# olydis/vlg_matching

Hardware: AMD Instinct MI355X
Metric: vlg_queries_per_sec (higher is better)
Workload: dtype u32

## Files before the change

### vlg_matching_amd/csrc/join_device.hpp

```cpp
#pragma once
#include "doc_cut.hpp"
namespace {

constexpr uint32_t kNone = 0xFFFFFFFFu;
constexpr uint32_t kChecksumSlots = 64;

struct SegMeta {
    uint32_t begin, end;
    uint32_t pbegin, pend;
    uint32_t dist;
    uint32_t level;
    uint32_t next;
    uint32_t query;
    uint64_t lo, hi;
};

struct QueryMeta {
    uint32_t seg0;
    uint32_t k;
    uint64_t end_len;
    uint64_t out_first;
    uint64_t out_tuple;
};

// ... 42 lines not shown
{
    RungLayout L{};
    L.levels = 0;
    while (L.levels < kMaxRungs && (total >> (kRungShift * (L.levels + 1))) != 0) ++L.levels;
    uint64_t at = 0;
    for (uint32_t j = 1; j <= L.levels; ++j) {
        L.off[j] = at;
        at += (((total >> (kRungShift * j)) + kRungFan - 1) & ~(uint64_t)(kRungFan - 1)) + kRungFan;
    }
    L.entries = at;
    return L;
}

template <typename pos_t>
__global__ void rung_build_kernel(const pos_t* __restrict__ P, uint64_t total, pos_t* __restrict__ R, const uint64_t* __restrict__ off, uint32_t levels,
                                  pos_t* __restrict__ F)
{
    for (uint64_t i = (uint64_t)blockIdx.x * blockDim.x + threadIdx.x; i < (total >> kRungShift); i += (uint64_t)gridDim.x * blockDim.x) {
        const pos_t v = P[kRungFan * i + kRungFan - 1];
        R[off[1] + i] = v;
        uint64_t k = i;
        for (uint32_t j = 2; j <= levels && (k & (kRungFan - 1)) == kRungFan - 1; ++j) {
            k >>= kRungShift;
            R[off[j] + k] = v;
            if (F && kRungShift * j == 6) F[k] = v;
        }
    }
}
constexpr bool kRungsHoldFences = 6 % kRungShift == 0 && kRungShift < 6;

template <typename pos_t> struct alignas(4 * sizeof(pos_t)) RungQuad { pos_t v[4]; };

constexpr uint32_t kFarRounds = 4;
template <typename pos_t>
__device__ __forceinline__ void wave_far_lower_bound(const pos_t* __restrict__ P, const pos_t* __restrict__ F, uint32_t wb, uint32_t b, pos_t key,
                                                     bool need, uint32_t& j, pos_t& val)
{
    const uint32_t lane = threadIdx.x & 63;
    constexpr pos_t kInf = (pos_t)~(pos_t)0;
    for (uint32_t round = 0; round < kFarRounds && wb < b; ++round) {
        if (!__any(need)) return;
        const uint32_t g0 = F ? wb >> 6 : 0;
        pos_t f;
        if (F) f = g0 + lane < (b >> 6) ? F[g0 + lane] : kInf;
        else { const uint64_t fi = (uint64_t)wb + 64 * lane + 63; f = fi < b ? P[fi] : kInf; }
        const pos_t flast = __shfl(f, 63);
        const bool can = need && key <= flast;
        uint32_t lo = 0;
#pragma unroll
        for (uint32_t step = 32; step; step >>= 1) {
            const pos_t v = __shfl(f, (int)(lo + step - 1));
            lo += v < key ? step : 0u;
        }
        if (can) {
            uint64_t w0 = F ? ((uint64_t)(g0 + lo) << 6) : (uint64_t)wb + 64 * lo;
            const uint64_t w1 = w0 + 64 < b ? w0 + 64 : b;
            if (w0 < wb) w0 = wb;
            uint32_t pos = 0;
#pragma unroll
            for (uint32_t step = 32; step; step >>= 1) {
                const uint64_t at = w0 + pos + step - 1;
                if (at < w1 && P[at] < key) pos += step;
            }
            const uint64_t at = w0 + pos;
            if (at < b) { j = (uint32_t)at; val = P[at]; } else j = b;
            need = false;
        }
        const uint64_t nwb = F ? ((uint64_t)(g0 + 64) << 6) : (uint64_t)wb + 4096;
        wb = nwb < b ? (uint32_t)nwb : b;
    }
    if (need) {
        j = gallop_lower_bound(P, wb < b ? wb : b, b, (uint64_t)key);
        if (j < b) val = P[j]; else j = b;
    }
// ... 1 lines not shown

constexpr uint32_t kCoopWindows = 4;
template <typename pos_t>
__device__ __forceinline__ uint32_t wave_lower_bound(const pos_t* __restrict__ P, const pos_t* __restrict__ F, uint32_t wb, uint32_t b, pos_t key, bool need, pos_t& val)
{
    const uint32_t lane = threadIdx.x & 63;
    constexpr pos_t kInf = (pos_t)~(pos_t)0;
    uint32_t res = b;
    for (uint32_t it = 0; it < kCoopWindows; ++it) {
        if (!__any(need)) break;
        const uint32_t idx = wb + lane;
        const pos_t w = idx < b ? P[idx] : kInf;
        const pos_t wlast = __shfl(w, 63);
        const bool can = need && key <= wlast;
        uint32_t lo = 0;
#pragma unroll
        for (uint32_t step = 32; step; step >>= 1) {
            const pos_t v = __shfl(w, (int)(lo + step - 1));
            lo += v < key ? step : 0u;
        }
        const pos_t at = __shfl(w, (int)lo);
        if (can) { res = wb + lo; val = at; need = false; }
        wb += 64;
    }
    if (__any(need)) wave_far_lower_bound(P, F, wb < b ? wb : b, b, key, need, res, val);
    return res < b ? res : b;
}

#ifndef VLG_COOP_WINDOWS2
#define VLG_COOP_WINDOWS2 4
#endif
static_assert(VLG_COOP_WINDOWS2 >= 1, "VLG_COOP_WINDOWS2: at least one window before the far search");
constexpr uint32_t kCoopWindows2 = VLG_COOP_WINDOWS2;
template <typename pos_t>
__device__ __forceinline__ void wave_lower_bound2(const pos_t* __restrict__ P, const pos_t* __restrict__ F, uint32_t wb, uint32_t b, pos_t key0, bool need0, pos_t key1,
                                                  bool need1, uint32_t& j0, pos_t& v0, uint32_t& j1, pos_t& v1)
{
    const uint32_t lane = threadIdx.x & 63;
    constexpr pos_t kInf = (pos_t)~(pos_t)0;
    j0 = b; j1 = b;
    for (uint32_t it = 0; it < kCoopWindows2; ++it) {
        if (!__any(need0 || need1)) break;
        const uint32_t idx = wb + lane;
        const pos_t w = idx < b ? P[idx] : kInf;
        const pos_t wlast = __shfl(w, 63);
        const bool can0 = need0 && key0 <= wlast, can1 = need1 && key1 <= wlast;
        uint32_t lo0 = 0, lo1 = 0;
#pragma unroll
        for (uint32_t step = 32; step; step >>= 1) {
            const pos_t a0 = __shfl(w, (int)(lo0 + step - 1)), a1 = __shfl(w, (int)(lo1 + step - 1));
            lo0 += a0 < key0 ? step : 0u;
            lo1 += a1 < key1 ? step : 0u;
        }
        const pos_t at0 = __shfl(w, (int)lo0), at1 = __shfl(w, (int)lo1);
        if (can0) { j0 = wb + lo0; v0 = at0; need0 = false; }
        if (can1) { j1 = wb + lo1; v1 = at1; need1 = false; }
        wb += 64;
    }
    if (__any(need0 || need1)) {
        wb = wb < b ? wb : b;
        wave_far_lower_bound(P, F, wb, b, key0, need0, j0, v0);
        wave_far_lower_bound(P, F, wb, b, key1, need1, j1, v1);
    }
}

constexpr uint32_t kKeys = 8;
constexpr uint32_t kBlk = 64 * kKeys;
constexpr uint32_t kTB = 1024;
constexpr uint32_t kKeyGroup = 4;
constexpr uint32_t kMinPiece = 128;

__device__ __forceinline__ void wave_sync()
{
    __builtin_amdgcn_fence(__ATOMIC_ACQ_REL, "wavefront");
    __builtin_amdgcn_wave_barrier();
}

template <typename T>
__device__ __forceinline__ T wave_min(T v)
{
    for (int o = 32; o > 0; o >>= 1) { const T u = __shfl_xor(v, o); v = u < v ? u : v; }
    return v;
}

template <typename T>
__device__ __forceinline__ T wave_max(T v)
{
    for (int o = 32; o > 0; o >>= 1) { const T u = __shfl_xor(v, o); v = u > v ? u : v; }
    return v;
}
template <typename T>
__device__ __forceinline__ T wave_or(T v)
{
    for (int o = 32; o > 0; o >>= 1) v |= __shfl_xor(v, o);
    return v;
// ... 380 lines not shown
    pos_t x_pre = 0, x_pre1 = 0;
    bool have_pre = false, have_pre1 = false;
    for (uint32_t base = run_begin; base < run_end; base += 64) {
        if (base >= seg_end) {
            while (seg_begin[s_w + 1] <= base) ++s_w;
            seg_end = seg_begin[s_w + 1];
            m = sm[s_w]; nx = sm[m.next];
            lvl0 = kJump && m.level == 0;
            end_len = lvl0 ? qm[m.query].end_len : 0;
            if (kDocs) { m_len = dr.seg_len[s_w]; m_next = dr.seg_len[m.next]; }
            have_pre = false; have_pre1 = false;
        }
        if (run_end - base >= 128 && base + 127 < seg_end) {
            const uint32_t e0 = base + lane, e1 = e0 + 64;
            const pos_t x0 = have_pre ? x_pre : P[phys_of(m, e0)];
            const pos_t x1 = have_pre1 ? x_pre1 : P[phys_of(m, e1)];
            const uint32_t left = run_end - base - 128;
            const uint32_t room = seg_end - base - 128;
            have_pre = left > 0 && (left < 64 ? left : 64u) <= room;
            have_pre1 = left >= 128 && room >= 128;
            if (lvl0) {
                x_pre = e0 + 128 < m.end ? P[phys_of(m, e0 + 128)] : kInf;
                x_pre1 = e1 + 128 < m.end ? P[phys_of(m, e1 + 128)] : kInf;
            } else {
                if (have_pre) x_pre = e0 + 128 < run_end ? P[phys_of(m, e0 + 128)] : (pos_t)0;
                if (have_pre1) x_pre1 = P[phys_of(m, e1 + 128)];
            }
            pos_t tlo0, thi0, tlo1, thi1, v0 = 0, v1 = 0;
            const bool want0 = gap_window<pos_t>((uint64_t)x0, nx.lo, nx.hi, tlo0, thi0);
            const bool want1 = gap_window<pos_t>((uint64_t)x1, nx.lo, nx.hi, tlo1, thi1);
            uint32_t j0 = nx.pend, j1 = nx.pend;
            if (hint_seg != s_w)
                hint = wave_kary_lower_bound(P, F, nx.pbegin, nx.pend, (uint64_t)__shfl(tlo0, 0));
            wave_lower_bound2(P, F, hint, nx.pend, tlo0, want0, tlo1, want1, j0, v0, j1, v1);
            if (!want0) j0 = nx.pend;
            if (!want1) j1 = nx.pend;
            bool in0 = want0, in1 = want1;
            uint64_t nb0 = 0, nb1 = 0;
            if (kDocs) {
                dw.locate(dr, (uint64_t)__shfl(x0, 0), (uint64_t)__shfl(x1, 63));
                nb0 = dw.nb(dr, (uint64_t)x0); nb1 = dw.nb(dr, (uint64_t)x1);
                in0 = want0 && doc_window<pos_t>((uint64_t)x0, m_len, m_next, nb0, thi0);
                in1 = want1 && doc_window<pos_t>((uint64_t)x1, m_len, m_next, nb1, thi1);
            }
            pos_t end0 = 0, end1 = 0;
            const bool ok0 = link_finish<pos_t, kLast>(P, nx, fb, e0, in0, j0, v0, thi0, endp, link, !lvl0, end0);
            const bool ok1 = link_finish<pos_t, kLast>(P, nx, fb, e1, in1, j1, v1, thi1, endp, link, !lvl0, end1);
            const unsigned long long okm0 = __ballot(ok0), okm1 = __ballot(ok1);
            if (lane == 0) { fbits_out[base >> 6] = okm0; fbits_out[(base >> 6) + 1] = okm1; }
            if (kJump) {
                if (lvl0) {
                    pos_t key[2] = {0, 0};
                    const bool need[2] = {ok0 && restart_key<pos_t, kDocs>((uint64_t)end0, end_len, nb0, key[0]),
                                          ok1 && restart_key<pos_t, kDocs>((uint64_t)end1, end_len, nb1, key[1])};
                    tile[lane] = x0; tile[64 + lane] = x1; tile[128 + lane] = x_pre; tile[192 + lane] = x_pre1;
                    wave_sync();
                    uint32_t out[2];
                    stretch_jump_targets<pos_t, 2>(P, F, m, phys_of(m, base), tile, key, need, out);
                    wave_sync();
                    jump[e0] = out[0]; jump[e1] = out[1];
                } else {
                    if (e0 >= jlo && e0 < jhi) jump[e0] = kNone;
                    if (e1 >= jlo && e1 < jhi) jump[e1] = kNone;
                }
            }
            hint_seg = s_w;
            hint = __shfl(j1, 63);
// ... 320 lines not shown
#pragma unroll
    for (uint32_t r = 0; r < 4; ++r) {
        const uint32_t li = threadIdx.x + 256 * r;
        const uint64_t e = base + li;
        if (e < r1) xh[e] = make_uint2(s_ext[st[r] >> 21], ((st[r] >> 11) & 1023u) + 1);
    }
}

__global__ void chain_walk_kernel(const SegMeta* __restrict__ sm, const QueryMeta* __restrict__ qm, uint32_t nq, FeasRef fb,
                                  const uint2* __restrict__ xh, const uint32_t* __restrict__ rec_begin,
                                  uint2* __restrict__ records, uint32_t* __restrict__ rec_count, unsigned long long* __restrict__ counts)
{
    uint32_t q = blockIdx.x * blockDim.x + threadIdx.x;
    if (q >= nq) return;
    const QueryMeta Q = qm[q];
    unsigned long long n_match = 0;
    uint32_t nrec = 0;
    if (Q.seg0 != kNone) {
        const uint32_t mbegin = sm[Q.seg0].begin, mend = sm[Q.seg0].end;
        uint2* rec = records + rec_begin[q];
        uint32_t cur = mbegin < mend ? next_feasible(fb, mbegin) : kNone;
        if (cur >= mend) cur = kNone;
        while (cur != kNone) {
            uint2 v = xh[cur];
            rec[nrec++] = make_uint2(cur, mbegin + (uint32_t)n_match);
            n_match += v.y;
            cur = v.x;
        }
    }
    rec_count[q] = nrec;
    counts[q] = n_match;
}

__global__ void __launch_bounds__(256) chain_emit_kernel(const uint32_t* __restrict__ rec_begin, const uint32_t* __restrict__ rec_count,
                                                         const uint2* __restrict__ records, uint32_t total_rec_slots,
                                                         const uint32_t* __restrict__ rec_query, const uint32_t* __restrict__ jump,
                                                         const uint2* __restrict__ xh, uint64_t r1 ,
                                                         uint32_t* __restrict__ mlist)
{
    constexpr uint16_t kOut = 0xFFFFu;
    constexpr uint32_t kPer = kTile / 64;
    __shared__ uint16_t s_t[4][2][kTile];
    const uint32_t lane = threadIdx.x & 63, wv = threadIdx.x >> 6;
    const uint32_t r = uniform((uint32_t)(((uint64_t)blockIdx.x * blockDim.x + threadIdx.x) >> 6));
    if (r >= total_rec_slots) return;
    const uint32_t q = rec_query[r];
    if (r - rec_begin[q] >= rec_count[q]) return;
    const uint2 rc = records[r];
    const uint64_t tile_base = (uint64_t)(rc.x / kTile) * kTile;
    const uint32_t cnt = uniform(xh[rc.x].y);
#pragma unroll
    for (uint32_t i = 0; i < kPer; ++i) {
        const uint64_t e = tile_base + lane + 64 * i;
        const uint32_t j = e < r1 ? jump[e] : kNone;
        s_t[wv][0][lane + 64 * i] = (j != kNone && (uint64_t)j < tile_base + kTile) ? (uint16_t)(j - (uint32_t)tile_base) : kOut;
    }
    wave_sync();
    uint32_t cur[kPer];
#pragma unroll
    for (uint32_t i = 0; i < kPer; ++i) cur[i] = rc.x - (uint32_t)tile_base;
    uint32_t buf = 0;
    for (uint32_t k = 0; (1u << k) < cnt; ++k) {
        const uint16_t* __restrict__ T = s_t[wv][buf];
#pragma unroll
        for (uint32_t i = 0; i < kPer; ++i) {
            const uint32_t rank = lane + 64 * i;
            if (rank < cnt && ((rank >> k) & 1)) cur[i] = T[cur[i]];
        }
        if ((2u << k) < cnt) {
            uint16_t* __restrict__ N = s_t[wv][buf ^ 1];
#pragma unroll
            for (uint32_t i = 0; i < kPer; ++i) {
                const uint32_t sl = lane + 64 * i;
                const uint16_t a = T[sl];
                N[sl] = a == kOut ? kOut : T[a];
            }
            wave_sync();
            buf ^= 1;
        }
    }
#pragma unroll
    for (uint32_t i = 0; i < kPer; ++i) {
        const uint32_t rank = lane + 64 * i;
        if (rank < cnt) mlist[rc.y + rank] = (uint32_t)tile_base + cur[i];
    }
}

template <typename pos_t>
__global__ void __launch_bounds__(256) join_gather_kernel(const pos_t* __restrict__ P, const SegMeta* __restrict__ sm, const QueryMeta* __restrict__ qm,
                                                          const unsigned long long* __restrict__ first_of , uint32_t nq,
                                                          uint64_t n_matches, const uint32_t* __restrict__ link, const uint32_t* __restrict__ mlist,
                                                          pos_t* __restrict__ out_first, pos_t* __restrict__ out_tuples, unsigned long long* __restrict__ checksum)
{
    const uint32_t lane = threadIdx.x & 63;
    const uint64_t wave = ((uint64_t)blockIdx.x * blockDim.x + threadIdx.x) >> 6;
    const uint64_t run_begin = wave * kRun;
    const bool live = run_begin < n_matches;
    const uint64_t run_end = !live ? run_begin : (run_begin + kRun < n_matches ? run_begin + kRun : n_matches);
    uint32_t q_w = 0, q_end = 0;
    if (live) {
        const uint32_t ub = wave_kary_lower_bound<unsigned long long>(first_of, 0, nq, run_begin + 1);
        q_w = uniform(ub ? ub - 1 : 0u);
        const uint32_t ue = wave_kary_lower_bound<unsigned long long>(first_of, 0, nq, run_end);
        q_end = uniform(ue ? ue - 1 : 0u);
    }
    unsigned long long local = 0;
    for (uint64_t base = run_begin; base < run_end; base += 64) {
        const uint64_t g = base + lane;
        uint32_t q = q_w;
        if (g < run_end) {
            uint32_t hi = q_end;
            while (q < hi) {
                const uint32_t mid = q + ((hi - q + 1) >> 1);
                if (first_of[mid] <= g) q = mid; else hi = mid - 1;
            }
            const QueryMeta Q = qm[q];
            const SegMeta m = sm[Q.seg0];
// ... 32 lines not shown
```

### vlg_matching_amd/csrc/search.hip

```cpp
#include <algorithm>
#include <chrono>
#include <cstdio>
#include <cstdlib>
#include <cstring>
#include <mutex>
#include <numeric>
#include <thread>
#include <unordered_map>
#include <string.h>
#include <string>
#include <vector>
#include "common.hpp"
#include "kernels.hpp"
#include <rocprim/rocprim.hpp>

using namespace vlg;

#include "search_types.hpp"
#include "filter_shape.hpp"
#include "window_cut.hpp"
#include "shape_dispatch.hpp"

enum { KS_BSEARCH = 0, KS_EXPAND, KS_LOCATE, KS_LOCATE_PART, KS_LOCATE_RESOLVE, KS_SORT, KS_FILTER_LADDER, KS_FILTER_PIVOT, KS_FILTER_PASS, KS_FILTER_COMPACT,
       KS_JOIN_INIT, KS_JOIN_LINK, KS_JOIN_SCAN, KS_JOIN_CHAIN, KS_GATHER, KS_EXCHANGE, KS_WINDOW_CUT, KS_CLASS_SEARCH, KS_COUNT };
static const char* kKernelNames[KS_COUNT] = {"backward_search", "expand", "locate", "locate_partition", "locate_resolve", "sort", "filter_ladder", "filter_pivot",
                                             "filter_pass", "filter_compact", "join_init", "join_link", "join_scan", "join_chain", "gather", "exchange", "window_cut", "class_search"};

struct vlg_workspace {
    hipStream_t stream = nullptr;
    uint64_t cap_bytes = 0;
    uint8_t* arena = nullptr;
    uint64_t arena_bytes = 0;
    HostPool host;
    bool profile = false;
    bool dedup = true;
    bool sweep = true;
    bool tuples = true;
    bool trail = true;
    bool filter = true;
    uint64_t filter_min = 1ull << 12;
    uint64_t filter_stream_min = 1ull << 16;
    bool filter_pivot = true;
    uint64_t filter_group_bytes = 0;
    uint64_t filter_pivot_ratio = 3;
    uint64_t pivot_range_ratio = 16;
    uint32_t compact_dense_min = 256;
    uint32_t pivot_rungs = 1;
    int list_sort = 1;
    uint64_t global_sort_min = 1ull << 20;
    bool quad_walk = true;
    bool fuse_jump = true;
    bool sweep_compact = true;
    uint64_t sweep_min = 1ull << 22;
    uint64_t sweep_tail = 1ull << 22;
    uint32_t unsample_pct = 0;
    uint64_t unsample_min = 1ull << 28;
    uint64_t unsample_tail = 1ull << 20;
    uint32_t class_intervals = 1024;
    uint64_t sample_reads = 0;
    uint8_t* head = nullptr;
    uint64_t head_bytes = 0;
    uint64_t tmp_key[6] = {0, 0, 0, 0, 0, 0};
    size_t tmp_bytes = 0;
    int x_ranks = 1, x_rank = 0;
    vlg_exchange_fn x_fn = nullptr;
    vlg_alltoall_fn x_a2a = nullptr;
    void* x_ctx = nullptr;
    void* x_comm = nullptr;
    bool exchange_all = false;
    uint64_t* x_status = nullptr;
    uint32_t x_agreed = 0;
    vlg_kernel_stat stats[KS_COUNT];
    std::vector<std::pair<hipEvent_t, hipEvent_t>> pending[KS_COUNT];
    std::vector<hipEvent_t> free_events;
};

namespace {

struct PhaseTrace {
    bool on, sync;
    hipStream_t st;
    std::chrono::steady_clock::time_point t0;
    explicit PhaseTrace(hipStream_t s) : on(getenv("VLG_TRACE") != nullptr), sync(!on || strcmp(getenv("VLG_TRACE"), "host") != 0), st(s), t0(std::chrono::steady_clock::now()) {}
    void mark(const char* what)
// ... 112 lines not shown

extern "C" void vlg_workspace_destroy(vlg_workspace* ws)
{
    if (!ws) return;
    ws_collect(ws);
    for (hipEvent_t e : ws->free_events) (void)hipEventDestroy(e);
    if (ws->arena) (void)hipFree(ws->arena);
    if (ws->head) (void)hipFree(ws->head);
    if (ws->x_status) (void)hipFree(ws->x_status);
    ws->host.release();
    delete ws;
}

extern "C" vlg_status vlg_workspace_profile(vlg_workspace* ws, int enable)
{
    if (!ws) return fail(VLG_E_INVALID, "null argument");
    ws_reset_stats(ws);
    ws->profile = enable != 0;
    return VLG_OK;
}

extern "C" vlg_status vlg_workspace_set_option(vlg_workspace* ws, const char* name, int64_t value)
{
    if (!ws || !name) return fail(VLG_E_INVALID, "null argument");
    if (!strcmp(name, "dedup")) { ws->dedup = value != 0; return VLG_OK; }
    if (!strcmp(name, "sweep")) { ws->sweep = value != 0; return VLG_OK; }
    if (!strcmp(name, "sweep_min")) { ws->sweep_min = (uint64_t)value; return VLG_OK; }
    if (!strcmp(name, "global_sort_min")) { ws->global_sort_min = (uint64_t)value; return VLG_OK; }
    if (!strcmp(name, "list_sort")) { ws->list_sort = value > 2 ? 1 : (int)value; return VLG_OK; }
    if (!strcmp(name, "trail")) { ws->trail = value != 0; return VLG_OK; }
    if (!strcmp(name, "quad_walk")) { ws->quad_walk = value != 0; return VLG_OK; }
    if (!strcmp(name, "tuples")) { ws->tuples = value != 0; return VLG_OK; }
    if (!strcmp(name, "fuse_jump")) { ws->fuse_jump = value != 0; return VLG_OK; }
    if (!strcmp(name, "sweep_compact")) { ws->sweep_compact = value != 0; return VLG_OK; }
    if (!strcmp(name, "filter")) { ws->filter = value != 0; return VLG_OK; }
    if (!strcmp(name, "filter_min")) { ws->filter_min = (uint64_t)value; return VLG_OK; }
    if (!strcmp(name, "filter_pivot")) { ws->filter_pivot = value != 0; return VLG_OK; }
    if (!strcmp(name, "filter_pivot_ratio")) { ws->filter_pivot_ratio = (uint64_t)value; return VLG_OK; }
    if (!strcmp(name, "pivot_range_ratio")) { ws->pivot_range_ratio = (uint64_t)std::max<int64_t>(0, value); return VLG_OK; }
    if (!strcmp(name, "compact_dense_min")) { ws->compact_dense_min = (uint32_t)std::max<int64_t>(0, std::min<int64_t>(value, 1 << 20)); return VLG_OK; }
    if (!strcmp(name, "pivot_rungs")) { ws->pivot_rungs = value <= 0 ? 0u : (value == 1 ? 1u : 2u); return VLG_OK; }
    if (!strcmp(name, "filter_stream_min")) { ws->filter_stream_min = (uint64_t)value; return VLG_OK; }
    if (!strcmp(name, "filter_group_bytes")) { ws->filter_group_bytes = (uint64_t)value; return VLG_OK; }
    if (!strcmp(name, "reserve")) {
        const uint64_t b = std::min<uint64_t>((uint64_t)value, ws->cap_bytes);
        return ws_reserve(ws, b + b / 96 + (256ull << 20));
    }
    if (!strcmp(name, "sweep_tail")) { ws->sweep_tail = (uint64_t)value; return VLG_OK; }
    if (!strcmp(name, "exchange_all")) { ws->exchange_all = value != 0; return VLG_OK; }
    if (!strcmp(name, "unsample_pct")) { ws->unsample_pct = (uint32_t)std::max<int64_t>(0, std::min<int64_t>(value, 1 << 20)); return VLG_OK; }
    if (!strcmp(name, "unsample_tail")) { ws->unsample_tail = (uint64_t)value; return VLG_OK; }
    if (!strcmp(name, "class_intervals")) {
        if (value < 1 || value > (int64_t)kClassIntervalsMax) return fail(VLG_E_INVALID, "class_intervals: 1 .. 2^20");
        ws->class_intervals = (uint32_t)value;
        return VLG_OK;
    }
    if (!strcmp(name, "unsample_min")) { ws->unsample_min = (uint64_t)value; return VLG_OK; }
    return fail(VLG_E_INVALID, std::string("unknown workspace option ") + name);
}

namespace {
vlg_status ws_exchange_reset(vlg_workspace* ws, int n_ranks)
{
    ws->x_comm = nullptr; ws->x_fn = nullptr; ws->x_a2a = nullptr; ws->x_ctx = nullptr; ws->x_ranks = 1; ws->x_rank = 0;
    if (n_ranks > 1 && !ws->x_status) VLG_HIP_TRY(hipMalloc((void**)&ws->x_status, 8 * 1024));
    return VLG_OK;
// ... 920 lines not shown
    if (vlg_status s = pp.carve()) return s;
    if (vlg_status s = pp.locate(plan_sort)) return s;
    if (vlg_status s = pp.sort(L.P)) return s;
    if (vlg_status s = pp.exchange(L.P, q, xq, ag)) return s;
    if (vlg_status s = pp.check_sort()) return s;
    if (vlg_status s = pp.fences_and_ladder()) return s;
    res->sum.located_occurrences += pp.acc;
    return VLG_OK;
}

}

#include "filter.hpp"

namespace {

inline bool fuse_jump_env() { static const bool on = [] { const char* e = getenv("VLG_FUSE_JUMP"); return !(e && e[0] == '0'); }(); return on; }

template <typename pos_t>
struct JoinChunk {
    const vlg_queries* q; vlg_workspace* ws; vlg_result* res; const uint64_t q0, q1; const Plan& pl; const Lists<pos_t>& L;
    Arena A;
    unsigned long long* d_stats; const FilterGroup* fg;
    hipStream_t st = ws->stream;
    PhaseTrace jt{st};
    const pos_t* P = L.P;
    pos_t* Pc = L.Pc;
    const pos_t* F = L.F;
    const uint64_t s0 = q->qsub[q0], s1 = q->qsub[q1];
    const uint32_t nseg = (uint32_t)(s1 - s0), nq = (uint32_t)(q1 - q0);
    ResultPiece piece{q0, q1};
    bool empty = false;
    const bool fused = ws->fuse_jump && fuse_jump_env();
    const vlg_documents* docs = q->docs;
    svec<uint64_t> seg_len; uint64_t* d_seglen = nullptr; DocRef dref{};
    svec<QueryMeta> qm;
    uint32_t kmax = 0, nlive = 0, n_rec = 0;
    svec<uint32_t> t_seg, t_cidx; svec<uint64_t> t_run0;
    bool t_kind[2] = {false, false};
    uint64_t pc_total = 0;
    std::vector<uint32_t> cls_count, cls_first;
    std::vector<uint64_t> cls_slot_begin, cls_slot_end;
    svec<SegMeta> sm; svec<uint32_t> seg_begin;
    uint64_t T = 0, lvl0_begin = 0, lvl0_end = 0, t0 = 0;
    svec<uint32_t> rec_begin, rec_query;
    svec<unsigned long long> counts, first_of;
    uint32_t* link = nullptr; pos_t* endp = nullptr;
    FeasBits fb; uint64_t* lvl_ptr[kBitLevels]; FeasBits* d_fb = nullptr; FeasRef fref{nullptr, nullptr};
    uint32_t* jump = nullptr; uint32_t* mlist = nullptr; uint2* xh = nullptr;
    SegMeta* d_sm = nullptr; QueryMeta* d_qm = nullptr; uint32_t* d_segb = nullptr; unsigned long long* d_counts = nullptr;
    uint32_t* d_recb = nullptr; uint32_t* d_recc = nullptr; uint32_t* d_recq = nullptr; uint2* d_rec = nullptr;

    uint64_t eo(uint64_t s) const { return fg ? fg->eff[s - fg->sub0] : pl.occ[s]; }
    bool filtered(uint64_t s) const { return fg && fg->cidx[s - fg->sub0] != kNone; }
    bool live(uint64_t qi) const { return q->qsub[qi + 1] > q->qsub[qi] && eo(q->qsub[qi]) > 0; }

    void survivor_tasks()
    {
        qm.resize(nq);
        if (fg) { t_seg.reserve(nseg); t_cidx.reserve(nseg); t_run0.reserve(nseg + 1); }
        t_run0.push_back(0);
        for (uint64_t qi = q0; qi < q1; ++qi) {
            const uint64_t a = q->qsub[qi];
            const uint32_t k = (uint32_t)(q->qsub[qi + 1] - a);
            QueryMeta& Q = qm[qi - q0];
            Q.k = k; Q.end_len = q->end_len[qi]; Q.out_first = Q.out_tuple = 0; Q.seg0 = kNone;
// ... 92 lines not shown
        sm[nlive] = SegMeta{(uint32_t)acc, (uint32_t)acc, 0, 0, 0, 0, kNone, 0, 0, 0};
        if (T == 0 || nlive == 0) { empty = true; return; }
        lvl0_begin = T; lvl0_end = 0;
        rec_begin.assign(nq + 1, 0);
        for (uint32_t i = 0; i < nq; ++i) {
            uint32_t cnt = 0;
            const SegMeta& m0 = sm[qm[i].seg0 != kNone ? qm[i].seg0 : nlive];
            if (m0.end > m0.begin) {
                lvl0_begin = std::min<uint64_t>(lvl0_begin, m0.begin); lvl0_end = std::max<uint64_t>(lvl0_end, m0.end);
                cnt = (m0.end - 1) / kTile - m0.begin / kTile + 1;
            }
            rec_begin[i + 1] = rec_begin[i] + cnt;
            rec_query.insert(rec_query.end(), cnt, i);
        }
        n_rec = rec_begin[nq];
        empty = lvl0_end <= lvl0_begin;
        t0 = lvl0_begin / kTile * kTile;
    }

    vlg_status carve()
    {
        link = ws->tuples ? A.take<uint32_t>(T) : nullptr;
        endp = A.take<pos_t>(T);
        uint64_t words = (T + 63) / 64 + 1;
        for (uint32_t l = 0; l < kBitLevels; ++l) {
            fb.lvl[l] = lvl_ptr[l] = A.take<uint64_t>(words);
            fb.words[l] = words;
            words = (words + 63) / 64 + 1;
        }
        d_fb = A.take<FeasBits>(1);
        fref = FeasRef{lvl_ptr[0], d_fb};
        const uint64_t n0 = lvl0_end - t0;
        uint32_t* jump_a = A.take<uint32_t>(n0);
        uint32_t* mlist_a = A.take<uint32_t>(n0);
        uint2* xh_a = A.take<uint2>(n0);
        jump = jump_a ? jump_a - t0 : nullptr;
        mlist = mlist_a ? mlist_a - t0 : nullptr;
        xh = xh_a ? xh_a - t0 : nullptr;
        d_sm = A.take<SegMeta>(nlive + 1);
        d_qm = A.take<QueryMeta>(nq);
        d_segb = A.take<uint32_t>(nlive + 2);
        if (docs) d_seglen = A.take<uint64_t>(nlive + 1);
        d_counts = A.take<unsigned long long>(nq);
        d_recb = A.take<uint32_t>(nq + 1);
        d_recc = A.take<uint32_t>(nq);
        d_recq = A.take<uint32_t>(n_rec + 1);
        d_rec = A.take<uint2>(n_rec + 1);
        if (A.failed) return fail(VLG_E_INTERNAL, "arena carve failed (join)");
        return VLG_OK;
    }

    vlg_status upload()
    {
        for (uint32_t l = 0; l < kBitLevels; ++l) VLG_HIP_TRY(hipMemsetAsync(lvl_ptr[l], 0, fb.words[l] * 8, st));
        VLG_HIP_TRY(hipMemcpyAsync(d_fb, &fb, sizeof fb, hipMemcpyHostToDevice, st));
        VLG_HIP_TRY(hipMemcpyAsync(d_recb, rec_begin.data(), (nq + 1) * 4, hipMemcpyHostToDevice, st));
        if (n_rec) VLG_HIP_TRY(hipMemcpyAsync(d_recq, rec_query.data(), n_rec * 4, hipMemcpyHostToDevice, st));
        VLG_HIP_TRY(hipMemcpyAsync(d_sm, sm.data(), (nlive + 1) * sizeof(SegMeta), hipMemcpyHostToDevice, st));
        VLG_HIP_TRY(hipMemcpyAsync(d_segb, seg_begin.data(), (nlive + 2) * 4, hipMemcpyHostToDevice, st));
        VLG_HIP_TRY(hipMemcpyAsync(d_qm, qm.data(), nq * sizeof(QueryMeta), hipMemcpyHostToDevice, st));
        if (docs) {
            VLG_HIP_TRY(hipMemcpyAsync(d_seglen, seg_len.data(), (nlive + 1) * 8, hipMemcpyHostToDevice, st));
            dref = doc_ref(docs, d_seglen);
        }
        return VLG_OK;
    }

// ... 9 lines not shown
        }
        VLG_HIP_TRY(hipGetLastError());
        return VLG_OK;
    }

    vlg_status link_classes()
    {
        if (cls_slot_end[0] > cls_slot_begin[0]) {
            Timed t(ws, KS_JOIN_INIT, 0);
            if (docs)
                hipLaunchKernelGGL(HIP_KERNEL_NAME(join_init_docs_kernel<pos_t>), dim3(runs_grid(cls_slot_end[0] - cls_slot_begin[0])), dim3(256), 0, st, P,
                                   d_segb, nlive, d_sm, cls_slot_begin[0], cls_slot_end[0], lvl_ptr[0], endp, dref);
            else
                hipLaunchKernelGGL(HIP_KERNEL_NAME(join_init_kernel<pos_t>), dim3(runs_grid(cls_slot_end[0] - cls_slot_begin[0])), dim3(256), 0, st, P,
                                   d_segb, nlive, d_sm, cls_slot_begin[0], cls_slot_end[0], lvl_ptr[0], endp);
        }
        if (vlg_status s = summarize_class(0)) return s;
        for (uint32_t dist = 1; dist < kmax; ++dist) {
            const uint64_t b0 = cls_slot_begin[dist], b1 = cls_slot_end[dist];
            if (b1 > b0) {
                const bool jumps = fused && b0 < lvl0_end && b1 > lvl0_begin;
                Timed t(ws, KS_JOIN_LINK, 8ull * (b1 - b0));
                const auto kernel = jumps ? (dist == 1 ? join_link_kernel<pos_t, true, true> : join_link_kernel<pos_t, false, true>)
                                          : (dist == 1 ? join_link_kernel<pos_t, true, false> : join_link_kernel<pos_t, false, false>);
                if (docs) {
                    const auto dkernel = jumps ? (dist == 1 ? join_link_docs_kernel<pos_t, true, true> : join_link_docs_kernel<pos_t, false, true>)
                                               : (dist == 1 ? join_link_docs_kernel<pos_t, true, false> : join_link_docs_kernel<pos_t, false, false>);
                    hipLaunchKernelGGL(dkernel, dim3(runs_grid(b1 - b0, kLinkRun)), dim3(256), 0, st, P, F, d_segb, nlive, d_sm, (uint32_t)b0, (uint32_t)b1,
                                       fref, lvl_ptr[0], endp, link, d_qm, (uint32_t)lvl0_begin, (uint32_t)lvl0_end, jump, dref);
                } else {
                    hipLaunchKernelGGL(kernel, dim3(runs_grid(b1 - b0, kLinkRun)), dim3(256), 0, st, P, F, d_segb, nlive, d_sm, (uint32_t)b0, (uint32_t)b1,
                                       fref, lvl_ptr[0], endp, link, d_qm, (uint32_t)lvl0_begin, (uint32_t)lvl0_end, jump);
                }
            }
            if (vlg_status s = summarize_class(dist)) return s;
        }
        return VLG_OK;
    }

    vlg_status chain()
    {
        {
            Timed t(ws, KS_JOIN_CHAIN, 8ull * (lvl0_end - lvl0_begin));
            const uint64_t jb = fused ? std::max(cls_slot_begin[0], lvl0_begin) : lvl0_begin, je = fused ? cls_slot_end[0] : lvl0_end;
            if (je > jb && docs)
                hipLaunchKernelGGL(HIP_KERNEL_NAME(join_jump_docs_kernel<pos_t>), dim3(runs_grid(je - jb)), dim3(256), 0, st, P, F, d_segb, nlive, d_sm, d_qm,
                                   jb, je, fref, endp, jump, dref);
            else if (je > jb)
                hipLaunchKernelGGL(HIP_KERNEL_NAME(join_jump_kernel<pos_t>), dim3(runs_grid(je - jb)), dim3(256), 0, st, P, F, d_segb, nlive, d_sm, d_qm, jb,
                                   je, fref, endp, jump);
            if (t0 < lvl0_begin) VLG_HIP_TRY(hipMemsetAsync(jump + t0, 0xFF, (lvl0_begin - t0) * 4, st));
            if (fused)
                for (uint32_t d = 1; d < kmax; ++d) {
                    const uint64_t p0 = std::max(cls_slot_end[d], lvl0_begin), p1 = std::min(cls_slot_begin[d - 1], lvl0_end);
                    if (p1 > p0) VLG_HIP_TRY(hipMemsetAsync(jump + p0, 0xFF, (p1 - p0) * 4, st));
                }
            hipLaunchKernelGGL(chain_tiles_kernel, dim3((uint32_t)((lvl0_end - t0 + kTile - 1) / kTile)), dim3(256), 0, st, jump, t0, lvl0_end, fref, d_segb,
                               nlive, xh);
            hipLaunchKernelGGL(chain_walk_kernel, dim3((nq + 63) / 64), dim3(64), 0, st, d_sm, d_qm, nq, fref, xh, d_recb, d_rec, d_recc, d_counts);
            if (n_rec)
                hipLaunchKernelGGL(chain_emit_kernel, dim3((n_rec + 3) / 4), dim3(256), 0, st, d_recb, d_recc, d_rec, n_rec, d_recq, jump, xh, lvl0_end, mlist);
        }
        VLG_HIP_TRY(hipGetLastError());
        return VLG_OK;
    }

    vlg_status gather()
    {
        counts.resize(nq);
        VLG_HIP_TRY(hipMemcpyAsync(counts.data(), d_counts, nq * 8, hipMemcpyDeviceToHost, st));
        VLG_HIP_TRY(hipStreamSynchronize(st));
        jt.mark("  chunk: link + chain");
        uint64_t M = 0, TV = 0;
        for (uint32_t i = 0; i < nq; ++i) {
            qm[i].out_first = M; qm[i].out_tuple = TV;
            M += counts[i]; TV += ws->tuples ? counts[i] * qm[i].k : 0;
            res->counts[q0 + i] = counts[i];
        }
        piece.matches = M; piece.tuple_vals = TV;
        if (M) {
            piece.width = sizeof(pos_t);
            VLG_HIP_TRY(result_alloc(&piece.d_first, M * sizeof(pos_t), &piece.first_bytes));
            if (TV) VLG_HIP_TRY(result_alloc(&piece.d_tuples, TV * sizeof(pos_t), &piece.tuple_bytes));
            res->pieces.push_back(piece);
            jt.mark("  chunk: result malloc");
            VLG_HIP_TRY(hipMemcpyAsync(d_qm, qm.data(), nq * sizeof(QueryMeta), hipMemcpyHostToDevice, st));
            first_of.resize(nq);
            for (uint32_t i = 0; i < nq; ++i) first_of[i] = qm[i].out_first;
            VLG_HIP_TRY(hipMemcpyAsync(d_counts, first_of.data(), nq * 8, hipMemcpyHostToDevice, st));
            Timed t(ws, KS_GATHER, sizeof(pos_t) * (M + TV));
            hipLaunchKernelGGL(HIP_KERNEL_NAME(join_gather_kernel<pos_t>), dim3(runs_grid(M)), dim3(256), 0, st, P, d_sm, d_qm, d_counts, nq, M, link, mlist,
                               static_cast<pos_t*>(piece.d_first), static_cast<pos_t*>(piece.d_tuples), d_stats + kStatsChecksum);
            VLG_HIP_TRY(hipGetLastError());
        } else {
            res->pieces.push_back(piece);
        }
        VLG_HIP_TRY(hipStreamSynchronize(st));
        jt.mark("  chunk: gather");
        res->sum.n_matches += M;
        res->sum.n_tuple_values += TV;
        res->sum.n_chunks++;
        res->sum.join_slots += T;
        return VLG_OK;
    }
};

template <typename pos_t>
vlg_status run_join_chunk(const vlg_queries* q, vlg_workspace* ws, vlg_result* res, uint64_t q0, uint64_t q1, const Plan& pl, const Lists<pos_t>& L,
                          const Arena& A, unsigned long long* d_stats, const FilterGroup* fg)
{
    JoinChunk<pos_t> jc{q, ws, res, q0, q1, pl, L, A, d_stats, fg};
    jc.survivor_tasks();
    if (vlg_status s = jc.compact_survivors()) return s;
    jc.jt.mark("  chunk: compaction launched");
    jc.layout();
    if (jc.empty) { res->pieces.push_back(jc.piece); return VLG_OK; }
    jc.jt.mark("  chunk: host metadata");
    if (vlg_status s = jc.carve()) return s;
    if (vlg_status s = jc.upload()) return s;
    if (vlg_status s = jc.link_classes()) return s;
    if (vlg_status s = jc.chain()) return s;
    return jc.gather();
}

struct JoinCost { uint64_t bytes, slots, survivors; };
// ... 892 lines not shown
        if (vlg_status s = ws_reserve(ws, list_bytes + jp.filter_need + jp.want_bytes + jp.meta + fixed)) return s;
        Arena A{ws->arena, ws->arena_bytes};
        L.P = A.take<uint64_t>(room.positions());
        uint64_t* F = A.take<uint64_t>(room.fence_entries);
        if (A.failed) return fail(VLG_E_INTERNAL, "arena carve failed (join lists)");
        if (total) VLG_HIP_TRY(hipMemcpyAsync(L.P, d_lists, total * 8, hipMemcpyDeviceToDevice, st));
        if (vlg_status s = wire_room_and_fences(L, room, total, F, st)) return s;
        tr.mark("join lists copied + checked");
        if (vlg_status s = run_joins<uint64_t>(n_positions, &qq, ws, res, pl, L, A, 0, n_joins, jp, d_stats, tr)) return s;
        unsigned long long hs[kStatsWords];
        return read_checksum(ws, res, d_stats, hs);
    };
    vlg_status stt;
    {
        HostPoolScope staging(&ws->host);
        try { stt = run(); }
        catch (const std::bad_alloc&) { stt = fail(VLG_E_OOM, "out of host memory while planning the joins (pinned staging)"); }
    }
    if (d_stats) (void)hipFree(d_stats);
    if (stt) { vlg_result_destroy(res); return stt; }
    *out = res;
    return VLG_OK;
}

#include "wtsa.hpp"
#include "wtsa_sdsl.hpp"
#include "int_index.hpp"

extern "C" vlg_status vlg_build_constants(vlg_build_constant* out, uint32_t cap, uint32_t* n)
{
    if (!n) return fail(VLG_E_INVALID, "null argument");
    const vlg::KernelConstants kc = vlg::kernel_constants();
    const struct { const char* name; int64_t value; } all[] = {
        {"VLG_LINK_RUN", VLG_LINK_RUN}, {"VLG_COOP_WINDOWS2", VLG_COOP_WINDOWS2}, {"VLG_RUNG_SHIFT", VLG_RUNG_SHIFT},
        {"VLG_RESOLVE_HOPS", kc.resolve_hops}, {"VLG_RESOLVE_CHUNK", kc.resolve_chunk}, {"VLG_GROUP_CHUNK", kc.group_chunk}, {"VLG_SWEEP_CHUNK", kc.sweep_chunk},
        {"VLG_STAGE_LISTS", kc.stage_lists}, {"VLG_SWEEP_PAIRS", kc.sweep_pairs},
        {"VLG_PIVOT_GROUPS", VLG_PIVOT_GROUPS}, {"VLG_PIVOT_TURNS", VLG_PIVOT_TURNS}, {"VLG_COMPACT_RUNS", VLG_COMPACT_RUNS},
        {"VLG_SPARSE_TURN", VLG_SPARSE_TURN}, {"VLG_SORT_CLASSES", VLG_SORT_CLASSES}, {"VLG_BUCKET_SORT", VLG_BUCKET_SORT},
        {"VLG_WINDOW_SORT", VLG_WINDOW_SORT}, {"VLG_WINDOWS_PER_TILE", VLG_WINDOWS_PER_TILE}, {"VLG_WINDOW_RANK_LOOP", VLG_WINDOW_RANK_LOOP},
        {"VLG_WINDOW_THREADS", VLG_WINDOW_THREADS}, {"VLG_WINDOW_ITEMS", VLG_WINDOW_ITEMS}, {"VLG_FETCH_THREADS", VLG_FETCH_THREADS},
        {"VLG_DOCLIST_RUN", VLG_DOCLIST_RUN},
    };
    const uint32_t count = (uint32_t)(sizeof(all) / sizeof(all[0]));
    *n = count;
    for (uint32_t i = 0; i < count && i < cap && out; ++i) {
        memset(out[i].name, 0, sizeof(out[i].name));
        strncpy(out[i].name, all[i].name, sizeof(out[i].name) - 1);
        out[i].value = all[i].value;
    }
    return VLG_OK;
}
```

### vlg_matching_amd/variants.py

```python
import os
import subprocess
from concurrent.futures import ThreadPoolExecutor

_HERE = os.path.dirname(os.path.abspath(__file__))
ROOT = os.path.dirname(_HERE)
CSRC = os.path.join(_HERE, "csrc")

DEFAULTS = {
    "VLG_LINK_RUN": 2048, "VLG_COOP_WINDOWS2": 4, "VLG_RUNG_SHIFT": 2, "VLG_RESOLVE_HOPS": 4096, "VLG_RESOLVE_CHUNK": 4096,
    "VLG_GROUP_CHUNK": 2048, "VLG_STAGE_LISTS": 1, "VLG_SWEEP_PAIRS": 1, "VLG_PIVOT_GROUPS": 2, "VLG_PIVOT_TURNS": 1,
    "VLG_COMPACT_RUNS": 16, "VLG_SPARSE_TURN": 8, "VLG_SORT_CLASSES": 5, "VLG_BUCKET_SORT": 1, "VLG_WINDOW_SORT": 1,
    "VLG_WINDOWS_PER_TILE": 2, "VLG_WINDOW_RANK_LOOP": 0, "VLG_WINDOW_THREADS": 256, "VLG_WINDOW_ITEMS": 12, "VLG_FETCH_THREADS": 16,
    "VLG_DOCLIST_RUN": 2048, "VLG_SWEEP_CHUNK": 2048,
}

VARIANTS = {
    "small": {"VLG_LINK_RUN": 192, "VLG_RESOLVE_CHUNK": 256, "VLG_GROUP_CHUNK": 256, "VLG_RESOLVE_HOPS": 2, "VLG_COMPACT_RUNS": 1,
              "VLG_SPARSE_TURN": 1, "VLG_PIVOT_GROUPS": 1, "VLG_COOP_WINDOWS2": 1, "VLG_DOCLIST_RUN": 192, "VLG_SWEEP_CHUNK": 512},
    "alternates": {"VLG_SORT_CLASSES": 3, "VLG_SWEEP_PAIRS": 0, "VLG_STAGE_LISTS": 0, "VLG_WINDOW_RANK_LOOP": 1, "VLG_WINDOWS_PER_TILE": 4,
                   "VLG_PIVOT_TURNS": 4, "VLG_RUNG_SHIFT": 4},
    "radix": {"VLG_BUCKET_SORT": 0, "VLG_RUNG_SHIFT": 3},
}

ENV_RUNS = {
    "env_paths": {"VLG_RESOLVE_GROUPED": "0", "VLG_SWEEP_LOOKAHEAD": "0", "VLG_NO_SPECULATIVE_COMPACT": "1", "VLG_WINDOW_SORT": "0",
                  "VLG_FUSE_JUMP": "0"},
}


def constants(name):
    c = dict(DEFAULTS)
    if name is not None:
        c.update(VARIANTS[name])
    return c


def extra_defs(name):
    return " ".join("-D%s=%d" % kv for kv in sorted(VARIANTS[name].items()))


def library(name):
    return os.path.join(ROOT, "build", "variants", name, "libvlg_hip.so")


def build(name, jobs=4):
    subprocess.check_call(["make", "-C", CSRC, "-j%d" % jobs, "variant", "VARIANT=" + name, "EXTRA_DEFS=" + extra_defs(name)],
                          stdout=subprocess.DEVNULL)


def build_all(jobs=None):
    jobs = jobs or max(1, min(8, (os.cpu_count() or 4) // len(VARIANTS)))
    with ThreadPoolExecutor(len(VARIANTS)) as ex:
        for f in [ex.submit(build, n, jobs) for n in VARIANTS]:
# ... 2 lines not shown
```

Baseline: 818,300.

## Emit first positions directly from chain walk and prefetch next link window

Adds a direct-emit path to the chain emit kernel. In the non-tuple case it writes first positions and checksum contributions straight to the output, so the intermediate mlist buffer and the separate gather kernel are no longer needed. The cooperative window search now also loads the next 64-element window one iteration ahead to hide global load latency. Optional link-search statistics counters are added behind a compile flag. The prefetch may issue a load that early exit never uses, and the checksum reduction adds a block-wide sync.

```diff
diff --git a/vlg_matching_amd/csrc/join_device.hpp b/vlg_matching_amd/csrc/join_device.hpp
--- a/vlg_matching_amd/csrc/join_device.hpp
+++ b/vlg_matching_amd/csrc/join_device.hpp
@@ -98,14 +98,23 @@
 template <typename pos_t> struct alignas(4 * sizeof(pos_t)) RungQuad { pos_t v[4]; };
 
 constexpr uint32_t kFarRounds = 4;
+
+#ifdef VLG_LINK_STATS
+enum { LS_PAIRS = 0, LS_WINDOWS, LS_PLACED, LS_FAR0, LS_FAR1, LS_FAR_ROUNDS0, LS_FAR_ROUNDS1, LS_COUNT };
+__device__ unsigned long long g_link_stats[LS_COUNT];
+#define VLG_LINK_STAT(i, n) do { const unsigned long long n_ = (unsigned long long)(n); if ((threadIdx.x & 63) == 0 && n_) atomicAdd(&g_link_stats[i], n_); } while (0)
+#else
+#define VLG_LINK_STAT(i, n) do { } while (0)
+#endif
 template <typename pos_t>
 __device__ __forceinline__ void wave_far_lower_bound(const pos_t* __restrict__ P, const pos_t* __restrict__ F, uint32_t wb, uint32_t b, pos_t key,
-                                                     bool need, uint32_t& j, pos_t& val)
+                                                     bool need, uint32_t& j, pos_t& val, uint32_t stat_reg = 2 )
 {
     const uint32_t lane = threadIdx.x & 63;
     constexpr pos_t kInf = (pos_t)~(pos_t)0;
     for (uint32_t round = 0; round < kFarRounds && wb < b; ++round) {
         if (!__any(need)) return;
+        if (stat_reg < 2) VLG_LINK_STAT(LS_FAR_ROUNDS0 + stat_reg, 1);
         const uint32_t g0 = F ? wb >> 6 : 0;
         pos_t f;
         if (F) f = g0 + lane < (b >> 6) ? F[g0 + lane] : kInf;
@@ -173,19 +182,34 @@
 #endif
 static_assert(VLG_COOP_WINDOWS2 >= 1, "VLG_COOP_WINDOWS2: at least one window before the far search");
 constexpr uint32_t kCoopWindows2 = VLG_COOP_WINDOWS2;
-template <typename pos_t>
+#ifndef VLG_LINK_EARLY
+#define VLG_LINK_EARLY 1
+#endif
+static_assert(VLG_LINK_EARLY == 0 || VLG_LINK_EARLY == 1, "VLG_LINK_EARLY: 0 or 1");
+template <typename pos_t, bool kEarly>
 __device__ __forceinline__ void wave_lower_bound2(const pos_t* __restrict__ P, const pos_t* __restrict__ F, uint32_t wb, uint32_t b, pos_t key0, bool need0, pos_t key1,
                                                   bool need1, uint32_t& j0, pos_t& v0, uint32_t& j1, pos_t& v1)
 {
     const uint32_t lane = threadIdx.x & 63;
     constexpr pos_t kInf = (pos_t)~(pos_t)0;
     j0 = b; j1 = b;
+    VLG_LINK_STAT(LS_PAIRS, 1);
+    pos_t w_next = kInf;
+    if (kEarly) w_next = wb + lane < b ? P[wb + lane] : kInf;
     for (uint32_t it = 0; it < kCoopWindows2; ++it) {
         if (!__any(need0 || need1)) break;
-        const uint32_t idx = wb + lane;
-        const pos_t w = idx < b ? P[idx] : kInf;
+        pos_t w;
+        if (kEarly) {
+            w = w_next;
+            if (it + 1 < kCoopWindows2) w_next = wb + 64 + lane < b ? P[wb + 64 + lane] : kInf;
+        } else {
+            const uint32_t idx = wb + lane;
+            w = idx < b ? P[idx] : kInf;
+        }
         const pos_t wlast = __shfl(w, 63);
         const bool can0 = need0 && key0 <= wlast, can1 = need1 && key1 <= wlast;
+        VLG_LINK_STAT(LS_WINDOWS, 1);
+        VLG_LINK_STAT(LS_PLACED, (__any(can0) ? 1 : 0) + (__any(can1) ? 1 : 0));
         uint32_t lo0 = 0, lo1 = 0;
 #pragma unroll
         for (uint32_t step = 32; step; step >>= 1) {
@@ -200,8 +224,10 @@
     }
     if (__any(need0 || need1)) {
         wb = wb < b ? wb : b;
-        wave_far_lower_bound(P, F, wb, b, key0, need0, j0, v0);
-        wave_far_lower_bound(P, F, wb, b, key1, need1, j1, v1);
+        VLG_LINK_STAT(LS_FAR0, __any(need0) ? 1 : 0);
+        VLG_LINK_STAT(LS_FAR1, __any(need1) ? 1 : 0);
+        wave_far_lower_bound(P, F, wb, b, key0, need0, j0, v0, 0);
+        wave_far_lower_bound(P, F, wb, b, key1, need1, j1, v1, 1);
     }
 }
 
@@ -648,7 +674,7 @@
             uint32_t j0 = nx.pend, j1 = nx.pend;
             if (hint_seg != s_w)
                 hint = wave_kary_lower_bound(P, F, nx.pbegin, nx.pend, (uint64_t)__shfl(tlo0, 0));
-            wave_lower_bound2(P, F, hint, nx.pend, tlo0, want0, tlo1, want1, j0, v0, j1, v1);
+            wave_lower_bound2<pos_t, VLG_LINK_EARLY != 0 && !(kDocs && sizeof(pos_t) == 8)>(P, F, hint, nx.pend, tlo0, want0, tlo1, want1, j0, v0, j1, v1);
             if (!want0) j0 = nx.pend;
             if (!want1) j1 = nx.pend;
             bool in0 = want0, in1 = want1;
@@ -1035,57 +1061,90 @@
     counts[q] = n_match;
 }
 
+template <typename pos_t, bool kDirect>
 __global__ void __launch_bounds__(256) chain_emit_kernel(const uint32_t* __restrict__ rec_begin, const uint32_t* __restrict__ rec_count,
                                                          const uint2* __restrict__ records, uint32_t total_rec_slots,
                                                          const uint32_t* __restrict__ rec_query, const uint32_t* __restrict__ jump,
                                                          const uint2* __restrict__ xh, uint64_t r1 ,
-                                                         uint32_t* __restrict__ mlist)
+                                                         uint32_t* __restrict__ mlist, const pos_t* __restrict__ P, const SegMeta* __restrict__ sm,
+                                                         const QueryMeta* __restrict__ qm, pos_t* __restrict__ out_first,
+                                                         unsigned long long* __restrict__ checksum)
 {
     constexpr uint16_t kOut = 0xFFFFu;
     constexpr uint32_t kPer = kTile / 64;
     __shared__ uint16_t s_t[4][2][kTile];
     const uint32_t lane = threadIdx.x & 63, wv = threadIdx.x >> 6;
     const uint32_t r = uniform((uint32_t)(((uint64_t)blockIdx.x * blockDim.x + threadIdx.x) >> 6));
-    if (r >= total_rec_slots) return;
-    const uint32_t q = rec_query[r];
-    if (r - rec_begin[q] >= rec_count[q]) return;
-    const uint2 rc = records[r];
-    const uint64_t tile_base = (uint64_t)(rc.x / kTile) * kTile;
-    const uint32_t cnt = uniform(xh[rc.x].y);
-#pragma unroll
-    for (uint32_t i = 0; i < kPer; ++i) {
-        const uint64_t e = tile_base + lane + 64 * i;
-        const uint32_t j = e < r1 ? jump[e] : kNone;
-        s_t[wv][0][lane + 64 * i] = (j != kNone && (uint64_t)j < tile_base + kTile) ? (uint16_t)(j - (uint32_t)tile_base) : kOut;
-    }
-    wave_sync();
-    uint32_t cur[kPer];
-#pragma unroll
-    for (uint32_t i = 0; i < kPer; ++i) cur[i] = rc.x - (uint32_t)tile_base;
-    uint32_t buf = 0;
-    for (uint32_t k = 0; (1u << k) < cnt; ++k) {
-        const uint16_t* __restrict__ T = s_t[wv][buf];
+    bool live = r < total_rec_slots;
+    uint32_t q = 0;
+    if (live) {
+        q = rec_query[r];
+        live = r - rec_begin[q] < rec_count[q];
+    }
+    unsigned long long local = 0;
+    if (live) {
+        const uint2 rc = records[r];
+        const uint64_t tile_base = (uint64_t)(rc.x / kTile) * kTile;
+        const uint32_t cnt = uniform(xh[rc.x].y);
 #pragma unroll
         for (uint32_t i = 0; i < kPer; ++i) {
-            const uint32_t rank = lane + 64 * i;
-            if (rank < cnt && ((rank >> k) & 1)) cur[i] = T[cur[i]];
-        }
-        if ((2u << k) < cnt) {
-            uint16_t* __restrict__ N = s_t[wv][buf ^ 1];
+            const uint64_t e = tile_base + lane + 64 * i;
+            const uint32_t j = e < r1 ? jump[e] : kNone;
+            s_t[wv][0][lane + 64 * i] = (j != kNone && (uint64_t)j < tile_base + kTile) ? (uint16_t)(j - (uint32_t)tile_base) : kOut;
+        }
+        wave_sync();
+        uint32_t cur[kPer];
+#pragma unroll
+        for (uint32_t i = 0; i < kPer; ++i) cur[i] = rc.x - (uint32_t)tile_base;
+        uint32_t buf = 0;
+        for (uint32_t k = 0; (1u << k) < cnt; ++k) {
+            const uint16_t* __restrict__ T = s_t[wv][buf];
 #pragma unroll
             for (uint32_t i = 0; i < kPer; ++i) {
-                const uint32_t sl = lane + 64 * i;
-                const uint16_t a = T[sl];
-                N[sl] = a == kOut ? kOut : T[a];
-            }
-            wave_sync();
-            buf ^= 1;
-        }
-    }
-#pragma unroll
-    for (uint32_t i = 0; i < kPer; ++i) {
-        const uint32_t rank = lane + 64 * i;
-        if (rank < cnt) mlist[rc.y + rank] = (uint32_t)tile_base + cur[i];
+                const uint32_t rank = lane + 64 * i;
+                if (rank < cnt && ((rank >> k) & 1)) cur[i] = T[cur[i]];
+            }
+            if ((2u << k) < cnt) {
+                uint16_t* __restrict__ N = s_t[wv][buf ^ 1];
+#pragma unroll
+                for (uint32_t i = 0; i < kPer; ++i) {
+                    const uint32_t sl = lane + 64 * i;
+                    const uint16_t a = T[sl];
+                    N[sl] = a == kOut ? kOut : T[a];
+                }
+                wave_sync();
+                buf ^= 1;
+            }
+        }
+        if (kDirect) {
+            const QueryMeta Q = qm[q];
+            const SegMeta m = sm[Q.seg0];
+            pos_t* const out = out_first + Q.out_first + (rc.y - m.begin);
+#pragma unroll
+            for (uint32_t i = 0; i < kPer; ++i) {
+                const uint32_t rank = lane + 64 * i;
+                if (rank < cnt) {
+                    const pos_t first = P[phys_of(m, (uint32_t)tile_base + cur[i])];
+                    out[rank] = first;
+                    local += first;
+                }
+            }
+        } else {
+#pragma unroll
+            for (uint32_t i = 0; i < kPer; ++i) {
+                const uint32_t rank = lane + 64 * i;
+                if (rank < cnt) mlist[rc.y + rank] = (uint32_t)tile_base + cur[i];
+            }
+        }
+    }
+    if (kDirect) {
+        __shared__ unsigned long long s_sum;
+        if (threadIdx.x == 0) s_sum = 0;
+        __syncthreads();
+        for (int o = 32; o > 0; o >>= 1) local += __shfl_down(local, o);
+        if (lane == 0 && local) atomicAdd(&s_sum, local);
+        __syncthreads();
+        if (threadIdx.x == 0 && s_sum) atomicAdd(checksum + (blockIdx.x % kChecksumSlots), s_sum);
     }
 }
 
diff --git a/vlg_matching_amd/csrc/search.hip b/vlg_matching_amd/csrc/search.hip
--- a/vlg_matching_amd/csrc/search.hip
+++ b/vlg_matching_amd/csrc/search.hip
@@ -50,6 +50,7 @@
     uint64_t global_sort_min = 1ull << 20;
     bool quad_walk = true;
     bool fuse_jump = true;
+    bool emit_direct = true;
     bool sweep_compact = true;
     uint64_t sweep_min = 1ull << 22;
     uint64_t sweep_tail = 1ull << 22;
@@ -228,6 +229,7 @@
     if (!strcmp(name, "quad_walk")) { ws->quad_walk = value != 0; return VLG_OK; }
     if (!strcmp(name, "tuples")) { ws->tuples = value != 0; return VLG_OK; }
     if (!strcmp(name, "fuse_jump")) { ws->fuse_jump = value != 0; return VLG_OK; }
+    if (!strcmp(name, "emit_direct")) { ws->emit_direct = value != 0; return VLG_OK; }
     if (!strcmp(name, "sweep_compact")) { ws->sweep_compact = value != 0; return VLG_OK; }
     if (!strcmp(name, "filter")) { ws->filter = value != 0; return VLG_OK; }
     if (!strcmp(name, "filter_min")) { ws->filter_min = (uint64_t)value; return VLG_OK; }
@@ -1214,6 +1216,7 @@
     ResultPiece piece{q0, q1};
     bool empty = false;
     const bool fused = ws->fuse_jump && fuse_jump_env();
+    const bool direct = !ws->tuples && ws->emit_direct;
     const vlg_documents* docs = q->docs;
     svec<uint64_t> seg_len; uint64_t* d_seglen = nullptr; DocRef dref{};
     svec<QueryMeta> qm;
@@ -1372,7 +1375,7 @@
         fref = FeasRef{lvl_ptr[0], d_fb};
         const uint64_t n0 = lvl0_end - t0;
         uint32_t* jump_a = A.take<uint32_t>(n0);
-        uint32_t* mlist_a = A.take<uint32_t>(n0);
+        uint32_t* mlist_a = direct ? nullptr : A.take<uint32_t>(n0);
         uint2* xh_a = A.take<uint2>(n0);
         jump = jump_a ? jump_a - t0 : nullptr;
         mlist = mlist_a ? mlist_a - t0 : nullptr;
@@ -1448,6 +1451,14 @@
                     hipLaunchKernelGGL(kernel, dim3(runs_grid(b1 - b0, kLinkRun)), dim3(256), 0, st, P, F, d_segb, nlive, d_sm, (uint32_t)b0, (uint32_t)b1,
                                        fref, lvl_ptr[0], endp, link, d_qm, (uint32_t)lvl0_begin, (uint32_t)lvl0_end, jump);
                 }
+#ifdef VLG_LINK_STATS
+                unsigned long long ls[LS_COUNT] = {0}, zero[LS_COUNT] = {0};
+                VLG_HIP_TRY(hipMemcpyFromSymbol(ls, HIP_SYMBOL(g_link_stats), sizeof ls));
+                VLG_HIP_TRY(hipMemcpyToSymbol(HIP_SYMBOL(g_link_stats), zero, sizeof zero));
+                fprintf(stderr, "[vlg link stats] width %d dist %u slots %llu pairs %llu windows %llu placed %llu far0 %llu far1 %llu "
+                                "far_rounds0 %llu far_rounds1 %llu\n", (int)sizeof(pos_t), dist, (unsigned long long)(b1 - b0), ls[LS_PAIRS],
+                        ls[LS_WINDOWS], ls[LS_PLACED], ls[LS_FAR0], ls[LS_FAR1], ls[LS_FAR_ROUNDS0], ls[LS_FAR_ROUNDS1]);
+#endif
             }
             if (vlg_status s = summarize_class(dist)) return s;
         }
@@ -1474,8 +1485,9 @@
             hipLaunchKernelGGL(chain_tiles_kernel, dim3((uint32_t)((lvl0_end - t0 + kTile - 1) / kTile)), dim3(256), 0, st, jump, t0, lvl0_end, fref, d_segb,
                                nlive, xh);
             hipLaunchKernelGGL(chain_walk_kernel, dim3((nq + 63) / 64), dim3(64), 0, st, d_sm, d_qm, nq, fref, xh, d_recb, d_rec, d_recc, d_counts);
-            if (n_rec)
-                hipLaunchKernelGGL(chain_emit_kernel, dim3((n_rec + 3) / 4), dim3(256), 0, st, d_recb, d_recc, d_rec, n_rec, d_recq, jump, xh, lvl0_end, mlist);
+            if (n_rec && !direct)
+                hipLaunchKernelGGL(HIP_KERNEL_NAME(chain_emit_kernel<pos_t, false>), dim3((n_rec + 3) / 4), dim3(256), 0, st, d_recb, d_recc, d_rec, n_rec,
+                                   d_recq, jump, xh, lvl0_end, mlist, nullptr, nullptr, nullptr, nullptr, nullptr);
         }
         VLG_HIP_TRY(hipGetLastError());
         return VLG_OK;
@@ -1501,12 +1513,18 @@
             res->pieces.push_back(piece);
             jt.mark("  chunk: result malloc");
             VLG_HIP_TRY(hipMemcpyAsync(d_qm, qm.data(), nq * sizeof(QueryMeta), hipMemcpyHostToDevice, st));
-            first_of.resize(nq);
-            for (uint32_t i = 0; i < nq; ++i) first_of[i] = qm[i].out_first;
-            VLG_HIP_TRY(hipMemcpyAsync(d_counts, first_of.data(), nq * 8, hipMemcpyHostToDevice, st));
-            Timed t(ws, KS_GATHER, sizeof(pos_t) * (M + TV));
-            hipLaunchKernelGGL(HIP_KERNEL_NAME(join_gather_kernel<pos_t>), dim3(runs_grid(M)), dim3(256), 0, st, P, d_sm, d_qm, d_counts, nq, M, link, mlist,
-                               static_cast<pos_t*>(piece.d_first), static_cast<pos_t*>(piece.d_tuples), d_stats + kStatsChecksum);
+            if (direct) {
+                Timed t(ws, KS_JOIN_CHAIN, sizeof(pos_t) * M);
+                hipLaunchKernelGGL(HIP_KERNEL_NAME(chain_emit_kernel<pos_t, true>), dim3((n_rec + 3) / 4), dim3(256), 0, st, d_recb, d_recc, d_rec, n_rec,
+                                   d_recq, jump, xh, lvl0_end, nullptr, P, d_sm, d_qm, static_cast<pos_t*>(piece.d_first), d_stats + kStatsChecksum);
+            } else {
+                first_of.resize(nq);
+                for (uint32_t i = 0; i < nq; ++i) first_of[i] = qm[i].out_first;
+                VLG_HIP_TRY(hipMemcpyAsync(d_counts, first_of.data(), nq * 8, hipMemcpyHostToDevice, st));
+                Timed t(ws, KS_GATHER, sizeof(pos_t) * (M + TV));
+                hipLaunchKernelGGL(HIP_KERNEL_NAME(join_gather_kernel<pos_t>), dim3(runs_grid(M)), dim3(256), 0, st, P, d_sm, d_qm, d_counts, nq, M, link,
+                                   mlist, static_cast<pos_t*>(piece.d_first), static_cast<pos_t*>(piece.d_tuples), d_stats + kStatsChecksum);
+            }
             VLG_HIP_TRY(hipGetLastError());
         } else {
             res->pieces.push_back(piece);
@@ -2465,7 +2483,7 @@
     if (!n) return fail(VLG_E_INVALID, "null argument");
     const vlg::KernelConstants kc = vlg::kernel_constants();
     const struct { const char* name; int64_t value; } all[] = {
-        {"VLG_LINK_RUN", VLG_LINK_RUN}, {"VLG_COOP_WINDOWS2", VLG_COOP_WINDOWS2}, {"VLG_RUNG_SHIFT", VLG_RUNG_SHIFT},
+        {"VLG_LINK_RUN", VLG_LINK_RUN}, {"VLG_COOP_WINDOWS2", VLG_COOP_WINDOWS2}, {"VLG_LINK_EARLY", VLG_LINK_EARLY}, {"VLG_RUNG_SHIFT", VLG_RUNG_SHIFT},
         {"VLG_RESOLVE_HOPS", kc.resolve_hops}, {"VLG_RESOLVE_CHUNK", kc.resolve_chunk}, {"VLG_GROUP_CHUNK", kc.group_chunk}, {"VLG_SWEEP_CHUNK", kc.sweep_chunk},
         {"VLG_STAGE_LISTS", kc.stage_lists}, {"VLG_SWEEP_PAIRS", kc.sweep_pairs},
         {"VLG_PIVOT_GROUPS", VLG_PIVOT_GROUPS}, {"VLG_PIVOT_TURNS", VLG_PIVOT_TURNS}, {"VLG_COMPACT_RUNS", VLG_COMPACT_RUNS},
diff --git a/vlg_matching_amd/variants.py b/vlg_matching_amd/variants.py
--- a/vlg_matching_amd/variants.py
+++ b/vlg_matching_amd/variants.py
@@ -11,14 +11,14 @@
     "VLG_GROUP_CHUNK": 2048, "VLG_STAGE_LISTS": 1, "VLG_SWEEP_PAIRS": 1, "VLG_PIVOT_GROUPS": 2, "VLG_PIVOT_TURNS": 1,
     "VLG_COMPACT_RUNS": 16, "VLG_SPARSE_TURN": 8, "VLG_SORT_CLASSES": 5, "VLG_BUCKET_SORT": 1, "VLG_WINDOW_SORT": 1,
     "VLG_WINDOWS_PER_TILE": 2, "VLG_WINDOW_RANK_LOOP": 0, "VLG_WINDOW_THREADS": 256, "VLG_WINDOW_ITEMS": 12, "VLG_FETCH_THREADS": 16,
-    "VLG_DOCLIST_RUN": 2048, "VLG_SWEEP_CHUNK": 2048,
+    "VLG_DOCLIST_RUN": 2048, "VLG_SWEEP_CHUNK": 2048, "VLG_LINK_EARLY": 1,
 }
 
 VARIANTS = {
     "small": {"VLG_LINK_RUN": 192, "VLG_RESOLVE_CHUNK": 256, "VLG_GROUP_CHUNK": 256, "VLG_RESOLVE_HOPS": 2, "VLG_COMPACT_RUNS": 1,
               "VLG_SPARSE_TURN": 1, "VLG_PIVOT_GROUPS": 1, "VLG_COOP_WINDOWS2": 1, "VLG_DOCLIST_RUN": 192, "VLG_SWEEP_CHUNK": 512},
     "alternates": {"VLG_SORT_CLASSES": 3, "VLG_SWEEP_PAIRS": 0, "VLG_STAGE_LISTS": 0, "VLG_WINDOW_RANK_LOOP": 1, "VLG_WINDOWS_PER_TILE": 4,
-                   "VLG_PIVOT_TURNS": 4, "VLG_RUNG_SHIFT": 4},
+                   "VLG_PIVOT_TURNS": 4, "VLG_RUNG_SHIFT": 4, "VLG_LINK_EARLY": 0},
     "radix": {"VLG_BUCKET_SORT": 0, "VLG_RUNG_SHIFT": 3},
 }
 
```

New measurement: 831,300 (median of 6 runs). 1.6% higher.
